# facebookresearch/param

Hardware: AMD Instinct MI355X
Metric: EmbeddingBag lookups/s + achieved HBM GB/s; all-to-all bus-BW at 1/2/4/8 GPU (higher is better)
Workload: dtype f32

## Files before the change

param_amd/csrc/bwd_sorted_apply_impl.inc:

```
__device__ __forceinline__ u32x4 raw16_load(const char* p, int pol) {
    const PM_GLOBAL u32x4* q = as_global<u32x4>(p);
    if (pol == 2) return *reinterpret_cast<const volatile PM_GLOBAL u32x4*>(q);
    return (pol == 1 || pol == 4) ? __builtin_nontemporal_load(q) : *q;
}
__device__ __forceinline__ void raw16_store(char* p, const u32x4 v, int pol) {
    PM_GLOBAL u32x4* q = as_global<u32x4>(p);
#ifdef PM_VISIBLE_STORES
    if (pol == 2) *reinterpret_cast<volatile PM_GLOBAL u32x4*>(q) = v;
    else if (pol >= 3) __hip_atomic_store(reinterpret_cast<PM_GLOBAL uint32_t*>(q), v.x, __ATOMIC_RELAXED, __HIP_MEMORY_SCOPE_AGENT),
                       __hip_atomic_store(reinterpret_cast<PM_GLOBAL uint32_t*>(q) + 1, v.y, __ATOMIC_RELAXED, __HIP_MEMORY_SCOPE_AGENT),
                       __hip_atomic_store(reinterpret_cast<PM_GLOBAL uint32_t*>(q) + 2, v.z, __ATOMIC_RELAXED, __HIP_MEMORY_SCOPE_AGENT),
                       __hip_atomic_store(reinterpret_cast<PM_GLOBAL uint32_t*>(q) + 3, v.w, __ATOMIC_RELAXED, __HIP_MEMORY_SCOPE_AGENT);
    else if (pol == 1) __builtin_nontemporal_store(v, q);
    else *q = v;
    return;
#endif
    if (pol == 2) asm volatile("global_store_dwordx4 %0, %1, off sc0 sc1\n\ts_nop 1" : : "v"(q), "v"(v) : "memory");
    else if (pol >= 3) asm volatile("global_store_dwordx4 %0, %1, off sc1\n\ts_nop 1" : : "v"(q), "v"(v) : "memory");
    else if (pol == 1) asm volatile("global_store_dwordx4 %0, %1, off nt\n\ts_nop 1" : : "v"(q), "v"(v) : "memory");
    else asm volatile("global_store_dwordx4 %0, %1, off\n\ts_nop 1" : : "v"(q), "v"(v) : "memory");
}
__device__ __forceinline__ void hidden_store16(float* p, const float (&a)[4]) {
    const u32x4 v = {__float_as_uint(a[0]), __float_as_uint(a[1]), __float_as_uint(a[2]), __float_as_uint(a[3])};
#ifdef PM_VISIBLE_STORES
// ... 169 lines not shown
        case 16: return launch_apply_w<DST, K, 16>(sp, stream);
        case 32: return launch_apply_w<DST, K, 32>(sp, stream);
        default: return launch_apply_w<DST, K, 64>(sp, stream);
    }
}


template <typename DST>
hipError_t launch_unique_g(const SortedParams& sp, const KParams& kp, const UniqueArgs& ua, int max_dim, hipStream_t stream) {
    unsigned n_wg = static_cast<unsigned>(kp.T) * static_cast<unsigned>(kp.tiles_per_table);
    if (sp.unique_wgs_per_cu > 0 && n_wg > 256u * static_cast<unsigned>(sp.unique_wgs_per_cu)) n_wg = 256u * static_cast<unsigned>(sp.unique_wgs_per_cu);
    const dim3 grid(n_wg), blk(kBlock);
    const size_t lds = tile_lds_bytes(kp.bags_per_block, kp.idx_cap, false);
    const int g = group_lanes(max_dim, DST::kVec);
    if (sp.mom && max_dim > g * DST::kVec) return hipErrorInvalidValue;
#define PM_LAUNCH_UNIQUE(G_)                                                                                                         \
    do {                                                                                                                             \
        if (sp.mom) hipLaunchKernelGGL((bwd_unique_kernel<DST, G_, 1>), grid, blk, lds, stream, sp, kp, ua.hyb_tab, ua.bloom, ua.emit_keys,  \
                                       ua.emit_vals, ua.key_bytes, ua.tile_cnt, ua.tile_cnt_stride, ua.bloom_wbits);                  \
        else hipLaunchKernelGGL((bwd_unique_kernel<DST, G_, 0>), grid, blk, lds, stream, sp, kp, ua.hyb_tab, ua.bloom, ua.emit_keys,         \
                                ua.emit_vals, ua.key_bytes, ua.tile_cnt, ua.tile_cnt_stride, ua.bloom_wbits);                         \
    } while (0)
    switch (g) {
        case 8: PM_LAUNCH_UNIQUE(8); break;
        case 16: PM_LAUNCH_UNIQUE(16); break;
        case 32: PM_LAUNCH_UNIQUE(32); break;
        default: PM_LAUNCH_UNIQUE(64); break;
    }
#undef PM_LAUNCH_UNIQUE
    return hipGetLastError();
}


template <typename DST>
hipError_t launch_rest_g(const SortedParams& sp, const KParams& kp, const RestArgs& ra, int max_dim, hipStream_t stream) {
    if (ra.T_h < 1 || ra.parts < 1) return hipErrorInvalidValue;
    const dim3 grid(static_cast<unsigned>(ra.T_h) * static_cast<unsigned>(ra.parts)), blk(kRestThreads);
    const size_t lds = static_cast<size_t>(2 * kRestCap + kRestAux) * sizeof(uint32_t);
    const int g = group_lanes(max_dim, DST::kVec);
    if (sp.mom && max_dim > g * DST::kVec) return hipErrorInvalidValue;
#define PM_LAUNCH_REST_O(G_, OPT_)                                                                                                  \
    do {                                                                                                                            \
        static const hipError_t attr_ = hipFuncSetAttribute(reinterpret_cast<const void*>(hyb_rest_kernel<DST, G_, OPT_>),          \
                                                            hipFuncAttributeMaxDynamicSharedMemorySize, static_cast<int>(lds));     \
        if (attr_ != hipSuccess) return attr_;                                                                                      \
        hipLaunchKernelGGL((hyb_rest_kernel<DST, G_, OPT_>), grid, blk, lds, stream, sp, kp, ra);                                   \
    } while (0)
#define PM_LAUNCH_REST(G_)                                                    \
    do {                                                                      \
        if (sp.mom) PM_LAUNCH_REST_O(G_, 1); else PM_LAUNCH_REST_O(G_, 0);    \
    } while (0)
    switch (g) {
        case 8: PM_LAUNCH_REST(8); break;
        case 16: PM_LAUNCH_REST(16); break;
        case 32: PM_LAUNCH_REST(32); break;
        default: PM_LAUNCH_REST(64); break;
    }
#undef PM_LAUNCH_REST
#undef PM_LAUNCH_REST_O
    return hipGetLastError();
}
```

param_amd/csrc/embbag_bwd_sorted_kernels.inc:

```

template <typename DST, int G>
__device__ __forceinline__ void adagrad_finish(char* wptr, float (&wrow)[DST::kVec], const float (&acc)[DST::kVec],
                                               bool any_col, float* mom_row, float mom_prev, int D, const SortedParams& p,
                                               int lig, int nt_rows, uint64_t rowkey, int c) {
    float ss = 0.0f;
    if (p.wd_mode == PM_WD_L2) {
#pragma unroll
        for (int k = 0; k < DST::kVec; ++k) {
            const float reg = any_col ? p.wd * wrow[k] : 0.0f;
            const float gx = acc[k] + reg;
            ss = ss + gx * gx;
        }
    } else {
#pragma unroll
        for (int k = 0; k < DST::kVec; ++k) ss = ss + acc[k] * acc[k];
    }
#pragma unroll
    for (int off = G / 2; off >= 1; off >>= 1) ss = ss + __shfl_xor(ss, off, G);
    const float m = mom_prev + ss / static_cast<float>(D);
    if (lig == 0) hidden_store4(mom_row, m);
    const float mult = p.lr / (sqrtf(m) + p.eps);
    if (any_col) {
        if (p.wd_mode != PM_WD_NONE) {
            const float shrink = p.wd_mode == PM_WD_L2 ? mult * p.wd : p.lr * p.wd;
// ... 821 lines not shown
    {
        const PM_GLOBAL uint32_t* sk = as_global<uint32_t>(ra.stage + static_cast<size_t>(t) * 2 * kRestCap);
        const PM_GLOBAL uint32_t* sv = sk + kRestCap;
#pragma unroll
        for (int r = 0; r < kRestItems; ++r) {
            const uint32_t off = static_cast<uint32_t>(r) * kWave + lane, pos = wave * chunk + off;
            const uint32_t e = (off < chunk && pos < n) ? pos : n - 1u;
            key[r] = sk[e];
            val[r] = sv[e];
        }
    }
    PM_STAMP_DRAINED(trace_id, 2);
    const int rounds = (bits + 7) / 8;
    uint32_t* const wcnt = s_aux + wave * 256;
    uint32_t* const s_dstart = s_aux + NW * 256;
    for (int rd = 0; rd < rounds; ++rd) {
        const int shift = 8 * rd;
        const int w = (bits - shift) < 8 ? (bits - shift) : 8;
        const uint32_t mask = (1u << w) - 1u;
        for (int i = threadIdx.x; i < NW * 256; i += kRestThreads) s_aux[i] = 0u;
        __syncthreads();
        uint32_t rank[kRestItems];
#pragma unroll
        for (int r = 0; r < kRestItems; ++r) {
            rank[r] = 0;
            if (static_cast<uint32_t>(r) * kWave < chunk) {
                const uint32_t off = static_cast<uint32_t>(r) * kWave + lane;
                const bool valid = off < chunk && wave * chunk + off < n;
                const uint32_t d = (key[r] >> shift) & mask;
                uint32_t below, total;
                match_digit<8>(d, valid, below, total);
                const uint32_t b0 = valid ? wcnt[d] : 0u;
                rank[r] = b0 + below;
                if (valid && below == 0) wcnt[d] = b0 + total;
            }
        }
        __syncthreads();
        uint32_t acc_d = 0;
        if (threadIdx.x < 256) {
#pragma unroll
            for (int ww = 0; ww < NW; ++ww) {
                const uint32_t c = s_aux[ww * 256 + threadIdx.x];
                s_aux[ww * 256 + threadIdx.x] = acc_d;
                acc_d += c;
            }
        }
        const uint32_t ex = rest_excl_scan<NW>(acc_d, s_tmp);
        if (threadIdx.x < 256) s_dstart[threadIdx.x] = ex;
        __syncthreads();
#pragma unroll
        for (int r = 0; r < kRestItems; ++r) {
            const uint32_t off = static_cast<uint32_t>(r) * kWave + lane;
            if (off < chunk && wave * chunk + off < n) {
                const uint32_t d = (key[r] >> shift) & mask;
                const uint32_t qp = s_dstart[d] + wcnt[d] + rank[r];
                s_key[qp] = key[r];
                s_val[qp] = val[r];
            }
        }
        __syncthreads();
        if (rd + 1 < rounds) {
#pragma unroll
            for (int r = 0; r < kRestItems; ++r) {
                const uint32_t off = static_cast<uint32_t>(r) * kWave + lane, pos = wave * chunk + off;
                if (off < chunk && pos < n) {
                    key[r] = s_key[pos];
                    val[r] = s_val[pos];
// ... 121 lines not shown
```

param_amd/csrc/seg_hybrid.inc:

```

#ifndef PM_MARK_THREADS
#define PM_MARK_THREADS 1024
#endif
constexpr int kMarkThreads = PM_MARK_THREADS;

constexpr int kPartMinSlices = 8;
constexpr int kPartItems = 8;
constexpr int kPartChunk = kMarkThreads * kPartItems;
__device__ __forceinline__ uint32_t part_cap(uint32_t count, int slices) { return count / static_cast<uint32_t>(slices / 2); }

template <int NB>
__global__ void __launch_bounds__(kMarkThreads) hyb_part_kernel(const SegDesc* desc, const HybTable* tab, const void* indices, int idx64, int T_h,
                                                                int64_t n_request, int slices, uint32_t* qa, uint32_t* qb, uint32_t* qtail) {
    constexpr int kW = kMarkThreads / kWave;
    __shared__ uint32_t s_start[kHybMaxTables], s_count[kHybMaxTables];
    __shared__ uint32_t s_sum;
    __shared__ uint32_t s_wcnt[kW][kBloomKMax], s_woff[kW][kBloomKMax], s_base[kBloomKMax];
    if (threadIdx.x == 0) s_sum = 0u;
    __syncthreads();
    {
        const int i = threadIdx.x;
        if (i < T_h) {
            const bool c = tab[i].cand != 0u;
            const SegDesc d = desc[i];
// ... 198 lines not shown
            int32_t v[U];
#pragma unroll
            for (int u = 0; u < U; ++u) {
                const uint32_t i = i0 + u * kMarkThreads + threadIdx.x;
                v[u] = ip[i < n ? i : last];
            }
#pragma unroll
            for (int u = 0; u < U; ++u) visit(static_cast<uint32_t>(v[u]), std::true_type{}, i0 + u * kMarkThreads + threadIdx.x < n);
        }
    }
    PM_STAMP(trace_id, 3);
    wave_lds_fence();
    if (static_cast<uint32_t>(lane) < q_tail - q_head) mark(ring[(q_head + lane) & (kRing - 1)]);
    __syncthreads();
    PM_STAMP(trace_id, 4);
    u32x4* out = reinterpret_cast<u32x4*>(bloom + (static_cast<size_t>(t) * slices + static_cast<size_t>(k)) * kBloomWords);
    const u32x4* d4 = reinterpret_cast<const u32x4*>(dup);
    for (int i = threadIdx.x; i < kBloomWords / 4; i += kMarkThreads) out[i] = d4[i];
    PM_STAMP_DRAINED(trace_id, 5);
}

__device__ __forceinline__ uint32_t bloom_flag(const uint32_t* tmap, uint32_t row, int wbits) {
    const uint32_t mask = bloom_mask(row);
    return (tmap[bloom_word(row, wbits)] & mask) == mask ? 1u : 0u;
}


constexpr int kStagePartsMin = 8, kStagePartsMax = 128;
inline int stage_parts(int tiles_per_table) {
    int p = tiles_per_table / 8;
    return p < kStagePartsMin ? kStagePartsMin : (p > kStagePartsMax ? kStagePartsMax : p);
}

template <typename K>
__global__ void __launch_bounds__(kT) hyb_stage_kernel(SegDesc* desc, HybTable* tab, int T_h, const uint32_t* tile_cnt, size_t cnt_stride,
                                                       HybTiles tl, const K* kb, const uint32_t* vb, K* ka, uint32_t* va, int parts,
                                                       int rest_enable, int tshift, uint32_t* stage, uint32_t* rest_n, uint32_t* stat) {
    __shared__ uint32_t s_tmp[kWaves];
    __shared__ uint32_t s_dst[kCompactMaxTiles + 1];
    const int t = blockIdx.x / parts, part = blockIdx.x % parts;
    if (t >= T_h) return;
    if (tab[t].mode != 1u) {
        if (part == 0 && threadIdx.x == 0) rest_n[t] = 0u;
        return;
    }
    const uint32_t nt = static_cast<uint32_t>(tl.tiles_per_table);
    const uint32_t* tc = tile_cnt + static_cast<size_t>(t) * cnt_stride;
    uint32_t carry = 0;
    for (uint32_t i0 = 0; i0 < nt; i0 += kT) {
        const uint32_t i = i0 + threadIdx.x;
        const uint32_t c = i < nt ? tc[i] : 0u;
        const uint32_t ex = block_excl_scan256(c, s_tmp);
        if (i < nt) s_dst[i] = carry + ex;
        carry += s_tmp[0] + s_tmp[1] + s_tmp[2] + s_tmp[3];
        __syncthreads();
    }
    if (threadIdx.x == 0) s_dst[nt] = carry;
    __syncthreads();
    const uint32_t total = s_dst[nt];
    const bool staged = rest_enable && total <= static_cast<uint32_t>(kRestCap);
    const uint64_t base = desc[t].in_start;
    const uint64_t per_tile = static_cast<uint64_t>(tl.bags_per_tile) * tab[t].pooling;
    const K row_mask = (static_cast<K>(1) << tshift) - 1;
    uint32_t* const st_k = stage + static_cast<size_t>(t) * 2 * kRestCap;
    uint32_t* const st_v = st_k + kRestCap;
    const uint32_t ga = static_cast<uint32_t>(static_cast<uint64_t>(nt) * part / parts), gb = static_cast<uint32_t>(static_cast<uint64_t>(nt) * (part + 1) / parts);
    const uint32_t e0 = s_dst[ga], e1 = s_dst[gb];
    for (uint32_t e = e0 + threadIdx.x; e < e1; e += kT) {
        uint32_t lo = ga, hi = gb;
        while (hi - lo > 1) {
            const uint32_t mid = (lo + hi) >> 1;
            if (s_dst[mid] <= e) lo = mid; else hi = mid;
// ... 24 lines not shown
```

param_amd/csrc/seg_sort.hip:

```cpp
#include <cstdlib>

#include "common.h"
#include "pm_experiments.h"

namespace pm {
namespace {

constexpr int kT = 256;
constexpr int kWaves = kT / kWave;
constexpr int kTile = kSegTile;
constexpr int kTileItems = kTile / kT;
constexpr int kRadix = 256;
constexpr int kRadixMax = 512;
constexpr uint32_t kWaveCap = 1024;
constexpr uint32_t kLocalCap = kTile;
constexpr int kL2Grid = 512;
constexpr int kBuildBags = 1024;
constexpr int kMaxLbPasses = 5;

struct SegHeader {
    uint32_t n_total;
    uint32_t n_tiles;
    uint32_t n_l2;
    uint32_t n_tiles2;
// ... 45 lines not shown
}


__device__ __forceinline__ uint32_t block_excl_scan256(uint32_t v, uint32_t* s_tmp) {
    const int lane = threadIdx.x % kWave, wave = threadIdx.x / kWave;
    uint32_t incl = v;
#pragma unroll
    for (int off = 1; off < kWave; off <<= 1) {
        const uint32_t up = __shfl_up(incl, off, kWave);
        if (lane >= off) incl += up;
    }
    if (lane == kWave - 1) s_tmp[wave] = incl;
    __syncthreads();
    uint32_t base = 0;
    for (int w = 0; w < wave; ++w) base += s_tmp[w];
    __syncthreads();
    return base + incl - v;
}


__global__ void __launch_bounds__(1024) seg_prep_tables_kernel(const void* indices, const void* offsets, int idx64, const int64_t* rows, int T,
                                                               int64_t B, int64_t N, int64_t bag_begin, int64_t bag_count, int force_ragged,
                                                               SegDesc* desc, uint32_t* zero4, const HybArgs hyb, HybTable* hyb_tab, uint32_t* qtail,
                                                               uint32_t* rest_stat) {
    __shared__ uint32_t s_sample[2048];
    __shared__ uint32_t s_rep;
    const int t = blockIdx.x;
    if (zero4 && t == 0 && threadIdx.x < 4) zero4[threadIdx.x] = 0u;
    if (t == 0 && threadIdx.x < 2) rest_stat[threadIdx.x] = 0u;
    if (qtail && t < kHybMaxTables && static_cast<int>(threadIdx.x) < hyb.slices) qtail[static_cast<size_t>(t) * hyb.slices + threadIdx.x] = 0u;
    const int64_t TB = static_cast<int64_t>(T) * B;
    const int64_t g0 = static_cast<int64_t>(t) * B + bag_begin;
    auto off_at = [&](int64_t g) -> int64_t { return g < TB ? load_index(offsets, g, idx64) : N; };
    const int64_t s = off_at(g0);
    const int64_t e = off_at(g0 + bag_count);
    const int64_t cnt = e > s ? e - s : 0;
    const int64_t L = (bag_count > 0 && cnt > 0 && cnt % bag_count == 0) ? cnt / bag_count : 0;
    int bad = (L == 0 || force_ragged) ? 1 : 0;
    const int64_t n_rows = rows[t];
    bool cand = t < kHybMaxTables && !bad && cnt >= kHybMinCount && cnt <= static_cast<int64_t>(hyb.slices) * (kHybMaxCount / kBloomK) &&
                cnt * 4 <= n_rows;
    const bool sample = cand && hyb.allow == 1;
    uint32_t sr[2] = {0u, 0u};
    if (sample) {
        const int64_t stride = cnt / 2048;
#pragma unroll
        for (int u = 0; u < 2; ++u) sr[u] = static_cast<uint32_t>(load_index(indices, s + (threadIdx.x + u * 1024) * stride, idx64));
        for (int i = threadIdx.x; i < 2048; i += 1024) s_sample[i] = 0u;
        if (threadIdx.x == 0) s_rep = 0u;
    }
    if (!bad) {
        for (int64_t i0 = threadIdx.x; i0 < bag_count; i0 += 8 * 1024) {
            int64_t v[8];
#pragma unroll
            for (int u = 0; u < 8; ++u) {
                const int64_t i = i0 + u * 1024;
                v[u] = i < bag_count ? off_at(g0 + i) : s + i * L;
            }
#pragma unroll
            for (int u = 0; u < 8; ++u)
                if (v[u] != s + (i0 + u * 1024) * L) bad = 1;
        }
    }
    bad = __syncthreads_or(bad);
    {
        cand = cand && !bad;
        if (sample) {
            uint32_t rep = 0;
#pragma unroll
            for (int u = 0; u < 2; ++u) {
                const uint32_t h = (sr[u] * 0x9E3779B1u) >> 16;
                rep += (atomicOr(&s_sample[h >> 5], 1u << (h & 31u)) >> (h & 31u)) & 1u;
            }
            if (rep) atomicAdd(&s_rep, rep);
            __syncthreads();
            cand = cand && s_rep * 8u <= 2048u;
        }
        if (threadIdx.x == 0) {
            HybTable h;
            h.mode = 0u;
            h.cand = (cand && hyb.allow) ? 1u : 0u;
            h.pooling = bad ? 0u : static_cast<uint32_t>(L);
            h.n_dup = 0u;
            hyb_tab[t] = h;
        }
    }
    if (threadIdx.x == 0) {
        SegDesc d;
        d.in_start = static_cast<uint32_t>(s);
        d.count = static_cast<uint32_t>(cnt);
        d.out_start = 0;
        d.pooling = bad ? 0u : static_cast<uint32_t>(L);
        d.tile_base = 0;
        d.ntiles = static_cast<uint32_t>((cnt + kTile - 1) / kTile);
        d.rbits = static_cast<uint32_t>(bits_for_dev(static_cast<uint64_t>(rows[t])));
        d.pad = 0;
        desc[t] = d;
    }
}

__device__ __forceinline__ void scan2_1024(uint32_t* s_a, uint32_t* s_b) {
    const int t = threadIdx.x;
    for (int off = 1; off < 1024; off <<= 1) {
        const uint32_t a = t >= off ? s_a[t - off] : 0u;
        const uint32_t b = t >= off ? s_b[t - off] : 0u;
        __syncthreads();
        s_a[t] += a;
        s_b[t] += b;
        __syncthreads();
    }
}

template <typename K, bool WEIGHTED>
__device__ __forceinline__ void build_keys_chunk(int t, int chunk, const void* indices, const void* offsets, int idx64, int T, int64_t B,
                                                 int64_t N, int64_t bag_begin, int64_t bag_count, const SegDesc* desc, int tshift, K* keys,
                                                 uint32_t* vals, uint32_t* bag_of, int64_t* s_off) {
    constexpr int kBags = kBuildBags;
    if (!WEIGHTED && (desc[t].pooling > 0 || desc[t].pad)) return;
    const int64_t bag0 = bag_begin + static_cast<int64_t>(chunk) * kBags;
    const int64_t left = bag_begin + bag_count - bag0;
    if (left <= 0) return;
    const int nb = left < kBags ? static_cast<int>(left) : kBags;
    const int64_t TB = static_cast<int64_t>(T) * B;
    const int64_t g0 = static_cast<int64_t>(t) * B + bag0;
    for (int i = threadIdx.x; i <= nb; i += blockDim.x) s_off[i] = (g0 + i < TB) ? load_index(offsets, g0 + i, idx64) : N;
    __syncthreads();
    const int64_t base = s_off[0], end = s_off[nb];
    for (int64_t j = base + threadIdx.x; j < end; j += blockDim.x) {
        int lo = 0, hi = nb;
        while (hi - lo > 1) {
            const int mid = (lo + hi) >> 1;
            if (s_off[mid] <= j) lo = mid; else hi = mid;
        }
        const uint32_t bag = static_cast<uint32_t>(bag0 + lo);
        keys[j] = (static_cast<K>(t) << tshift) | static_cast<K>(load_index(indices, j, idx64));
        if (WEIGHTED) {
            vals[j] = static_cast<uint32_t>(j);
            bag_of[j] = bag;
        } else {
            vals[j] = bag;
        }
    }
}

template <typename K, bool WEIGHTED>
__global__ void __launch_bounds__(1024) seg_prep_scan_kernel(SegDesc* desc, int T, SegHeader* hdr, TileDesc* tiles, uint32_t tiles_cap,
                                                             const void* indices, const void* offsets, int idx64, int64_t B, int64_t N,
                                                             int64_t bag_begin, int64_t bag_count, int tshift, K* keys, uint32_t* vals,
                                                             uint32_t* bag_of, int chunks_per_table) {
    __shared__ uint32_t s_cnt[1024], s_til[1024], s_tb[1025], s_out[1024];
    __shared__ int64_t s_off[kBuildBags + 1];
    if (blockIdx.x > 0) {
        const int w = static_cast<int>(blockIdx.x) - 1;
        build_keys_chunk<K, WEIGHTED>(w / chunks_per_table, w % chunks_per_table, indices, offsets, idx64, T, B, N, bag_begin, bag_count,
                                      desc, tshift, keys, vals, bag_of, s_off);
        return;
    }
    const int t = threadIdx.x;
    const uint32_t c = t < T ? desc[t].count : 0u;
    const uint32_t nt = t < T ? desc[t].ntiles : 0u;
    s_cnt[t] = c;
    s_til[t] = nt;
    __syncthreads();
    scan2_1024(s_cnt, s_til);
    const uint32_t out_start = s_cnt[t] - c, tile_base = s_til[t] - nt;
    const uint32_t n_total = s_cnt[1023], n_tiles = s_til[1023];
    __syncthreads();
    if (t < T) {
        desc[t].out_start = out_start;
        desc[t].tile_base = tile_base;
        s_tb[t] = tile_base;
        s_out[t] = out_start;
    }
    if (t == 0) {
        s_tb[T] = n_tiles;
        hdr->n_total = n_total;
        hdr->n_tiles = n_tiles;
        hdr->n_l2 = 0;
        hdr->n_tiles2 = 0;
        hdr->lookback_timeouts = 0;
    }
    __syncthreads();
    const uint32_t n_write = n_tiles < tiles_cap ? n_tiles : tiles_cap;
    for (uint32_t g = t; g < n_write; g += 1024) {
        int lo = 0, hi = T;
        while (hi - lo > 1) {
            const int mid = (lo + hi) >> 1;
            if (s_tb[mid] <= g) lo = mid; else hi = mid;
        }
        const SegDesc d = desc[lo];
        const uint32_t first = (g - s_tb[lo]) * static_cast<uint32_t>(kTile);
        TileDesc td;
        td.seg = static_cast<uint32_t>(lo);
        td.cnt = (d.count - first) < static_cast<uint32_t>(kTile) ? d.count - first : static_cast<uint32_t>(kTile);
        td.in_base = d.in_start + first;
        td.out_base = s_out[lo] + first;
        td.first = first;
        td.pooling = d.pooling;
        td.rbits = d.rbits;
        td.magic = d.pooling > 1 ? static_cast<uint32_t>(0x100000000ull / d.pooling) + 1u : 0u;
        tiles[g] = td;
    }
}

template <typename K>
struct PassSrc {
    const void* indices;
    int idx64;
    const K* keys;
    const uint32_t* vals;
    int first;
    int tshift;
    uint32_t bag_begin;
};

__device__ __forceinline__ void wave_hist_add(uint32_t* h, uint32_t dg, bool valid, int lane) {
    const uint64_t vmask = __ballot(valid);
    const uint32_t firstd = __builtin_amdgcn_readfirstlane(dg);
    const bool uniform = __ballot(valid && dg != firstd) == 0 && (vmask & 1ull);
    if (uniform) {
        if (lane == 0) atomicAdd(&h[firstd], static_cast<uint32_t>(__popcll(vmask)));
    } else if (valid) {
        atomicAdd(&h[dg], 1u);
    }
}

template <typename K>
__device__ __forceinline__ void load_tile_rows(const TileDesc& td, const PassSrc<K>& src, uint64_t (&row)[kTileItems]) {
    const uint32_t cnt = td.cnt, last = cnt - 1u;
    auto at = [&](int k) { const uint32_t q = k * kT + threadIdx.x; return q < cnt ? q : last; };
    if (src.first && td.pooling > 0) {
        if (src.idx64) {
            const PM_GLOBAL int64_t* ip = as_global<int64_t>(src.indices) + td.in_base;
#pragma unroll
            for (int k = 0; k < kTileItems; ++k) row[k] = static_cast<uint64_t>(ip[at(k)]);
// ... 343 lines not shown

__device__ __forceinline__ u32x4 load_status(const uint32_t* p) {
    u32x4 v;
    asm volatile("global_load_dwordx4 %0, %1, off sc1\n\ts_waitcnt vmcnt(0)" : "=&v"(v) : "v"(p) : "memory");
    return v;
}
#ifndef PM_LB_BATCH
#define PM_LB_BATCH 4
#endif
constexpr int kLbBatch = PM_LB_BATCH;
__device__ __forceinline__ void load_status_batch(const uint32_t* const (&p)[kLbBatch], u32x4 (&v)[kLbBatch]) {
#if PM_LB_BATCH == 8
    asm volatile(
        "global_load_dwordx4 %0, %8, off sc1\n\tglobal_load_dwordx4 %1, %9, off sc1\n\t"
        "global_load_dwordx4 %2, %10, off sc1\n\tglobal_load_dwordx4 %3, %11, off sc1\n\t"
        "global_load_dwordx4 %4, %12, off sc1\n\tglobal_load_dwordx4 %5, %13, off sc1\n\t"
        "global_load_dwordx4 %6, %14, off sc1\n\tglobal_load_dwordx4 %7, %15, off sc1\n\ts_waitcnt vmcnt(0)"
        : "=&v"(v[0]), "=&v"(v[1]), "=&v"(v[2]), "=&v"(v[3]), "=&v"(v[4]), "=&v"(v[5]), "=&v"(v[6]), "=&v"(v[7])
        : "v"(p[0]), "v"(p[1]), "v"(p[2]), "v"(p[3]), "v"(p[4]), "v"(p[5]), "v"(p[6]), "v"(p[7])
        : "memory");
#else
    asm volatile(
        "global_load_dwordx4 %0, %4, off sc1\n\tglobal_load_dwordx4 %1, %5, off sc1\n\t"
        "global_load_dwordx4 %2, %6, off sc1\n\tglobal_load_dwordx4 %3, %7, off sc1\n\ts_waitcnt vmcnt(0)"
        : "=&v"(v[0]), "=&v"(v[1]), "=&v"(v[2]), "=&v"(v[3])
        : "v"(p[0]), "v"(p[1]), "v"(p[2]), "v"(p[3])
        : "memory");
#endif
}
__device__ __forceinline__ void store_status(uint32_t* p, u32x4 v) {
    asm volatile("global_store_dwordx4 %0, %1, off sc1\n\ts_nop 1" : : "v"(p), "v"(v) : "memory");
}

template <typename K, int RB>
__global__ void __launch_bounds__(kT) seg_hist_all_kernel(const TileDesc* tiles, const uint32_t* n_tiles, const PassSrc<K> src, int npass,
                                                          uint32_t tiles_cap, uint32_t* st) {
    constexpr int RAD = 1 << RB;
    __shared__ uint32_t h[kMaxLbPasses * RAD];
    const TileDesc td = tiles[blockIdx.x];
    const uint32_t nt = *n_tiles;
    if (blockIdx.x >= nt) return;
    const uint32_t g = blockIdx.x, cnt = td.cnt;
    int shift[kMaxLbPasses];
    uint32_t mask[kMaxLbPasses];
#pragma unroll
    for (int p = 0; p < kMaxLbPasses; ++p) pass_digit(0, p, td.rbits, RB, shift[p], mask[p]);
    for (int i = threadIdx.x; i < npass * RAD; i += kT) h[i] = 0;
    __syncthreads();
    const int lane = threadIdx.x % kWave;
    uint64_t row[kTileItems];
    load_tile_rows<K>(td, src, row);
    constexpr uint32_t kNone = 0xffffffffu;
    uint32_t hot0[kMaxLbPasses], hot1[kMaxLbPasses];
#pragma unroll
    for (int p = 0; p < kMaxLbPasses; ++p) {
        hot0[p] = hot1[p] = kNone;
        if (p < npass) {
            const bool v0 = threadIdx.x < cnt;
            const uint32_t dg = static_cast<uint32_t>(row[0] >> shift[p]) & mask[p];
            uint64_t cand = __ballot(v0);
            for (int r = 0; r < 3 && cand != 0; ++r) {
                const int leader = __builtin_amdgcn_readfirstlane(__ffsll(static_cast<long long>(cand)) - 1);
                const uint32_t d0 = __builtin_amdgcn_readlane(dg, leader);
                const uint64_t same = __ballot(v0 && dg == d0);
                cand &= ~same;
                if (__popcll(same) >= 8) {
                    if (hot0[p] == kNone) hot0[p] = d0;
                    else if (hot1[p] == kNone) hot1[p] = d0;
                }
            }
        }
    }
    bool any_hot = false;
#pragma unroll
// ... 515 lines not shown
    return &scratch_layout(const_cast<void*>(scratch), n_max, T).hdr->n_total;
}
const uint32_t* seg_sort_timeouts(const void* scratch, size_t n_max, int T) {
    return &scratch_layout(const_cast<void*>(scratch), n_max, T).hdr->lookback_timeouts;
}
const HybTable* seg_sort_hyb_tab(const void* scratch, size_t n_max, int T) { return scratch_layout(const_cast<void*>(scratch), n_max, T).hyb_tab; }
const uint32_t* seg_sort_bloom(const void* scratch, size_t n_max, int T) { return scratch_layout(const_cast<void*>(scratch), n_max, T).bloom; }
uint32_t* seg_sort_tile_cnt(const void* scratch, size_t n_max, int T) { return scratch_layout(const_cast<void*>(scratch), n_max, T).tile_cnt; }
size_t seg_sort_tile_cnt_stride(size_t n_max) { return tile_cnt_stride(n_max); }
uint32_t* seg_sort_rest_stat(void* scratch, size_t n_max, int T) { return &scratch_layout(scratch, n_max, T).hdr->rest_pairs; }
const uint32_t* seg_sort_rest_stage(const void* scratch, size_t n_max, int T) { return scratch_layout(const_cast<void*>(scratch), n_max, T).rest_stage; }
const uint32_t* seg_sort_rest_n(const void* scratch, size_t n_max, int T) { return scratch_layout(const_cast<void*>(scratch), n_max, T).rest_n; }

int seg_sort_radix_bits(int mode, int rbits_max) {
    if ((mode != 0 && mode != 3) || rbits_max <= 8) return 8;
    return (rbits_max + 8) / 9 < (rbits_max + 7) / 8 ? 9 : 8;
}
int seg_sort_passes(int mode, int rbits_max) {
    if ((mode != 0 && mode != 3) || rbits_max <= 0) return 1;
    const int rb = seg_sort_radix_bits(mode, rbits_max);
    return (rbits_max + rb - 1) / rb;
}
bool seg_sort_result_in_b(int mode, int rbits_max) { return seg_sort_passes(mode, rbits_max) % 2 == 1; }

bool seg_sort_lookback(int mode, int rbits_max, int64_t n) {
    if (mode != 0 || n >= (1ll << 30)) return false;
    const int np = seg_sort_passes(mode, rbits_max);
    return np <= kMaxLbPasses && static_cast<size_t>(np) << seg_sort_radix_bits(mode, rbits_max) <= kLbRowWords;
}

namespace {
template <typename K, int RB>
void launch_lookback(const Scratch& s, unsigned tm, int T, PassSrc<K> src, int total, K* keys_a, K* keys_b, uint32_t* vals_a, uint32_t* vals_b,
                     uint32_t spin_cap, hipStream_t stream) {
    src.first = 1;
    src.keys = keys_a;
    src.vals = vals_a;
    hipLaunchKernelGGL((seg_hist_all_kernel<K, RB>), dim3(tm), dim3(kT), 0, stream, s.tiles, &s.hdr->n_tiles, src, total, tm, s.st_all);
    hipLaunchKernelGGL((seg_scan_all_kernel<RB>), dim3(T, total), dim3(kRadix * kScanChunks), 0, stream, s.desc, s.st_all, tm, T, s.bstart_all);
    for (int p = 0; p < total; ++p) {
        src.first = p == 0 ? 1 : 0;
        src.keys = p == 0 ? keys_a : (p % 2 == 1 ? keys_b : keys_a);
        src.vals = p == 0 ? vals_a : (p % 2 == 1 ? vals_b : vals_a);
        K* kout = (p % 2 == 0) ? keys_b : keys_a;
        uint32_t* vout = (p % 2 == 0) ? vals_b : vals_a;
        hipLaunchKernelGGL((seg_lookback_pass_kernel<K, RB>), dim3(tm), dim3(kT), 0, stream, s.tiles, s.hdr, src, p, T, tm, s.st_all, s.bstart_all,
                           kout, vout, spin_cap);
    }
}
template <typename K, int RB>
void launch_level1_pass(const Scratch& s, unsigned tm, int T, const PassSrc<K>& src, int mode, int p, K* kout, uint32_t* vout, hipStream_t stream) {
    hipLaunchKernelGGL((seg_hist_kernel<K, RB>), dim3(tm), dim3(kT), 0, stream, s.tiles, &s.hdr->n_tiles, src, mode, p, s.bh);
    hipLaunchKernelGGL((seg_scan_kernel<RB>), dim3(T), dim3(kRadix * kScanChunks), 0, stream, s.hdr, s.desc, static_cast<const uint32_t*>(nullptr),
                       static_cast<uint32_t>(T), s.bh, s.bstart, s.bcnt, (mode != 0 && p == 0) ? 1 : 0, mode, s.l2_list);
    hipLaunchKernelGGL((seg_scatter_kernel<K, RB>), dim3(tm), dim3(kT), 0, stream, s.tiles, &s.hdr->n_tiles, src, mode, p, s.bh, s.bstart, kout, vout);
}
}

bool seg_sort_hybrid_available() {
    static const bool ok = hipFuncSetAttribute(reinterpret_cast<const void*>(hyb_mark_kernel), hipFuncAttributeMaxDynamicSharedMemorySize,
                                               2 * kBloomWords * 4) == hipSuccess;
    return ok;
}

template <typename K>
hipError_t seg_sort_part_a(const SegSortRequest& rq, void* scratch, hipStream_t stream) {
    if (rq.N == 0) return hipSuccess;
    if (rq.T < 1 || rq.T > kSegSortMaxTables || rq.N > 0xffffffffLL) return hipErrorInvalidValue;
    const size_t n = static_cast<size_t>(rq.N);
    const Scratch s = scratch_layout(scratch, n, rq.T);
    HybArgs hyb = rq.hyb;
    if (rq.weighted) hyb.allow = 0;
    hipLaunchKernelGGL(seg_prep_tables_kernel, dim3(rq.T), dim3(1024), 0, stream, rq.indices, rq.offsets, rq.idx64, rq.rows, rq.T, rq.B, rq.N,
                       rq.bag_begin, rq.bag_count, rq.weighted ? 1 : 0, s.desc, rq.zero4, hyb, s.hyb_tab, hyb.allow ? s.qtail : nullptr,
                       &s.hdr->rest_pairs);
    if (hyb.allow) {
        if (!seg_sort_hybrid_available()) return hipErrorInvalidValue;
        const int th = rq.T < kHybMaxTables ? rq.T : kHybMaxTables;
        static const int part_env = [] { const char* e = getenv("PARAM_AMD_HYB_PART"); return e ? atoi(e) : -1; }();
        const bool part = rq.queue_a && rq.queue_b && part_env != 0 && (part_env == 1 || hyb.slices >= kPartMinSlices);
        if (part) {
            const unsigned pgrid = static_cast<unsigned>((rq.N + kPartChunk - 1) / kPartChunk);
#define PM_LAUNCH_PART(NB_)                                                                                                               \
    hipLaunchKernelGGL((hyb_part_kernel<NB_>), dim3(pgrid), dim3(kMarkThreads), 0, stream, s.desc, s.hyb_tab, rq.indices, rq.idx64, th, rq.N, \
                       hyb.slices, rq.queue_a, rq.queue_b, s.qtail)
            switch (hyb.slices) {
                case 4: PM_LAUNCH_PART(2); break;
                case 8: PM_LAUNCH_PART(3); break;
                case 16: PM_LAUNCH_PART(4); break;
                case 32: PM_LAUNCH_PART(5); break;
                default: PM_LAUNCH_PART(6); break;
            }
#undef PM_LAUNCH_PART
        }
        const unsigned grid = static_cast<unsigned>(kXcds * hyb.slices * ((th + kXcds - 1) / kXcds));
        hipLaunchKernelGGL(hyb_mark_kernel, dim3(grid), dim3(kMarkThreads), 2 * kBloomWords * 4, stream, s.desc, s.hyb_tab, rq.indices, rq.idx64, th,
                           rq.T, rq.N, s.bloom, hyb.slices, part ? rq.queue_a : nullptr, part ? rq.queue_b : nullptr, part ? s.qtail : nullptr);
    }
    return hipGetLastError();
}

template <typename K>
hipError_t seg_sort_stage_leftovers(const SegSortRequest& rq, const K* keys_b, const uint32_t* vals_b, K* keys_a, uint32_t* vals_a,
                                    HybTiles tiles, int rest_enable, void* scratch, hipStream_t stream) {
    if (rq.N == 0) return hipSuccess;
    if (rq.T < 1 || rq.T > kSegSortMaxTables || rq.N > 0xffffffffLL) return hipErrorInvalidValue;
    if (tiles.tiles_per_table < 1 || tiles.tiles_per_table > kCompactMaxTiles) return hipErrorInvalidValue;
    const size_t n = static_cast<size_t>(rq.N);
    const Scratch s = scratch_layout(scratch, n, rq.T);
    const int th = rq.T < kHybMaxTables ? rq.T : kHybMaxTables;
    const int parts = stage_parts(tiles.tiles_per_table);
    hipLaunchKernelGGL((hyb_stage_kernel<K>), dim3(th * parts), dim3(kT), 0, stream, s.desc, s.hyb_tab, th, s.tile_cnt, tile_cnt_stride(n), tiles,
                       keys_b, vals_b, keys_a, vals_a, parts, rest_enable, rq.tshift, s.rest_stage, s.rest_n, &s.hdr->rest_pairs);
    return hipGetLastError();
}

template <typename K>
hipError_t seg_sort_part_b(const SegSortRequest& rq, int mode, K* keys_a, K* keys_b, uint32_t* vals_a, uint32_t* vals_b, uint32_t* bag_of,
                           void* scratch, hipStream_t stream, bool hybrid_done) {
    if (rq.N == 0) return hipSuccess;
    if (rq.T < 1 || rq.T > kSegSortMaxTables || rq.N > 0xffffffffLL) return hipErrorInvalidValue;
    const size_t n = static_cast<size_t>(rq.N);
    const Scratch s = scratch_layout(scratch, n, rq.T);
    const unsigned tm = static_cast<unsigned>(tiles_max(n, rq.T));
    if (rq.hyb.allow && !rq.weighted && !hybrid_done) return hipErrorInvalidValue;
    {
        const int chunks = rq.bag_count > 0 ? static_cast<int>((rq.bag_count + kBuildBags - 1) / kBuildBags) : 0;
        const dim3 gp(1u + static_cast<unsigned>(chunks) * static_cast<unsigned>(rq.T));
        if (rq.weighted)
            hipLaunchKernelGGL((seg_prep_scan_kernel<K, true>), gp, dim3(1024), 0, stream, s.desc, rq.T, s.hdr, s.tiles, tm, rq.indices,
                               rq.offsets, rq.idx64, rq.B, rq.N, rq.bag_begin, rq.bag_count, rq.tshift, keys_a, vals_a, bag_of, chunks);
        else
            hipLaunchKernelGGL((seg_prep_scan_kernel<K, false>), gp, dim3(1024), 0, stream, s.desc, rq.T, s.hdr, s.tiles, tm, rq.indices,
                               rq.offsets, rq.idx64, rq.B, rq.N, rq.bag_begin, rq.bag_count, rq.tshift, keys_a, vals_a, bag_of, chunks);
    }
    const int total = seg_sort_passes(mode, rq.rbits_max), rb = seg_sort_radix_bits(mode, rq.rbits_max);
    const bool lookback = seg_sort_lookback(mode, rq.rbits_max, rq.N);
    if (mode == 3) mode = 0;
    PassSrc<K> src;
    src.indices = rq.indices;
    src.idx64 = rq.idx64;
    src.tshift = rq.tshift;
    src.bag_begin = static_cast<uint32_t>(rq.bag_begin);
    if (lookback) {
        const uint32_t cap = rq.spin_cap ? rq.spin_cap : kLbSpinCap;
        if (rb == 9) launch_lookback<K, 9>(s, tm, rq.T, src, total, keys_a, keys_b, vals_a, vals_b, cap, stream);
        else launch_lookback<K, 8>(s, tm, rq.T, src, total, keys_a, keys_b, vals_a, vals_b, cap, stream);
        return hipGetLastError();
    }
    for (int p = 0; p < total; ++p) {
        src.first = p == 0 ? 1 : 0;
        src.keys = p == 0 ? keys_a : (p % 2 == 1 ? keys_b : keys_a);
        src.vals = p == 0 ? vals_a : (p % 2 == 1 ? vals_b : vals_a);
        K* kout = (p % 2 == 0) ? keys_b : keys_a;
        uint32_t* vout = (p % 2 == 0) ? vals_b : vals_a;
        if (rb == 9) launch_level1_pass<K, 9>(s, tm, rq.T, src, mode, p, kout, vout, stream);
        else launch_level1_pass<K, 8>(s, tm, rq.T, src, mode, p, kout, vout, stream);
    }
    if (mode != 0 && rq.rbits_max > 8) {
        const uint32_t nb = static_cast<uint32_t>(rq.T) * kRadix;
        hipLaunchKernelGGL((seg_local_kernel<K>), dim3((nb + kWaves - 1) / kWaves), dim3(kT), 0, stream, s.desc, s.bstart, s.bcnt, nb, mode,
                           keys_b, vals_b);
        hipLaunchKernelGGL(seg_l2_prep_kernel, dim3(1), dim3(1024), 0, stream, s.hdr, s.desc, s.bstart, s.bcnt, s.l2_list, mode, s.desc2,
                           static_cast<uint32_t>(seg2_max(n)), s.tiles2, static_cast<uint32_t>(tiles2_max(n)));
        int p2 = (rq.rbits_max - 8 + 7) / 8;
        if (p2 % 2) ++p2;
        src.first = 0;
        for (int q = 0; q < p2; ++q) {
            src.keys = (q % 2 == 0) ? keys_b : keys_a;
            src.vals = (q % 2 == 0) ? vals_b : vals_a;
            K* kout = (q % 2 == 0) ? keys_a : keys_b;
            uint32_t* vout = (q % 2 == 0) ? vals_a : vals_b;
            hipLaunchKernelGGL((seg_hist_kernel<K, 8>), dim3(kL2Grid), dim3(kT), 0, stream, s.tiles2, &s.hdr->n_tiles2, src, 0, q, s.bh2);
            hipLaunchKernelGGL((seg_scan_kernel<8>), dim3(kL2Grid / 2), dim3(kRadix * kScanChunks), 0, stream, s.hdr, s.desc2, &s.hdr->n_l2, 0u, s.bh2, s.bstart2,
                               s.bcnt2, 0, 0, static_cast<uint32_t*>(nullptr));
            hipLaunchKernelGGL((seg_scatter_loop_kernel<K, 8>), dim3(kL2Grid), dim3(kT), 0, stream, s.tiles2, &s.hdr->n_tiles2, src, 0, q, s.bh2,
                               s.bstart2, kout, vout);
        }
    }
    return hipGetLastError();
// ... 25 lines not shown
```

Before: 21.86 billion.

## Fuse key-build into hybrid stage kernel and self-compute tile descriptors in histogram

Unweighted key-building work moves into extra blocks of the hybrid stage kernel. When lookback sort is used, the histogram kernel derives the tile descriptors itself through an in-block scan, so the separate prep/scan launch is dropped. This is meant to remove kernel launches and serialization in the sorted backward path. It also makes the shared-memory attribute cache per device, prefetches the first offsets in the pooling check, and adds LDS fences around the radix rank update. The cost is redundant per-block descriptor scans and more complex control flow; an environment variable can turn the fusion off.

```diff
diff --git a/param_amd/csrc/bwd_sorted_apply_impl.inc b/param_amd/csrc/bwd_sorted_apply_impl.inc
--- a/param_amd/csrc/bwd_sorted_apply_impl.inc
+++ b/param_amd/csrc/bwd_sorted_apply_impl.inc
@@ -225,6 +225,7 @@
 }
 
 
+constexpr int kRestAttrDevices = 64;
 template <typename DST>
 hipError_t launch_rest_g(const SortedParams& sp, const KParams& kp, const RestArgs& ra, int max_dim, hipStream_t stream) {
     if (ra.T_h < 1 || ra.parts < 1) return hipErrorInvalidValue;
@@ -232,11 +233,17 @@
     const size_t lds = static_cast<size_t>(2 * kRestCap + kRestAux) * sizeof(uint32_t);
     const int g = group_lanes(max_dim, DST::kVec);
     if (sp.mom && max_dim > g * DST::kVec) return hipErrorInvalidValue;
+    int dev = 0;
+    if (hipGetDevice(&dev) != hipSuccess || dev < 0) return hipErrorInvalidDevice;
 #define PM_LAUNCH_REST_O(G_, OPT_)                                                                                                  \
     do {                                                                                                                            \
-        static const hipError_t attr_ = hipFuncSetAttribute(reinterpret_cast<const void*>(hyb_rest_kernel<DST, G_, OPT_>),          \
-                                                            hipFuncAttributeMaxDynamicSharedMemorySize, static_cast<int>(lds));     \
-        if (attr_ != hipSuccess) return attr_;                                                                                      \
+        static unsigned char set_[kRestAttrDevices];                                                                                \
+        if (dev >= kRestAttrDevices || !__atomic_load_n(&set_[dev], __ATOMIC_ACQUIRE)) {                                            \
+            const hipError_t attr_ = hipFuncSetAttribute(reinterpret_cast<const void*>(hyb_rest_kernel<DST, G_, OPT_>),             \
+                                                         hipFuncAttributeMaxDynamicSharedMemorySize, static_cast<int>(lds));        \
+            if (attr_ != hipSuccess) return attr_;                                                                                  \
+            if (dev < kRestAttrDevices) __atomic_store_n(&set_[dev], static_cast<unsigned char>(1), __ATOMIC_RELEASE);              \
+        }                                                                                                                           \
         hipLaunchKernelGGL((hyb_rest_kernel<DST, G_, OPT_>), grid, blk, lds, stream, sp, kp, ra);                                   \
     } while (0)
 #define PM_LAUNCH_REST(G_)                                                    \
diff --git a/param_amd/csrc/embbag_bwd_sorted_kernels.inc b/param_amd/csrc/embbag_bwd_sorted_kernels.inc
--- a/param_amd/csrc/embbag_bwd_sorted_kernels.inc
+++ b/param_amd/csrc/embbag_bwd_sorted_kernels.inc
@@ -877,7 +877,9 @@
                 match_digit<8>(d, valid, below, total);
                 const uint32_t b0 = valid ? wcnt[d] : 0u;
                 rank[r] = b0 + below;
+                wave_lds_fence();
                 if (valid && below == 0) wcnt[d] = b0 + total;
+                wave_lds_fence();
             }
         }
         __syncthreads();
diff --git a/param_amd/csrc/seg_hybrid.inc b/param_amd/csrc/seg_hybrid.inc
--- a/param_amd/csrc/seg_hybrid.inc
+++ b/param_amd/csrc/seg_hybrid.inc
@@ -254,12 +254,29 @@
     return p < kStagePartsMin ? kStagePartsMin : (p > kStagePartsMax ? kStagePartsMax : p);
 }
 
+constexpr int kStageBuildBags = 256;
+struct StageBuild {
+    const void* indices;
+    const void* offsets;
+    int idx64, T, chunks;
+    int64_t B, N, bag_begin, bag_count;
+};
 template <typename K>
 __global__ void __launch_bounds__(kT) hyb_stage_kernel(SegDesc* desc, HybTable* tab, int T_h, const uint32_t* tile_cnt, size_t cnt_stride,
                                                        HybTiles tl, const K* kb, const uint32_t* vb, K* ka, uint32_t* va, int parts,
-                                                       int rest_enable, int tshift, uint32_t* stage, uint32_t* rest_n, uint32_t* stat) {
+                                                       int rest_enable, int tshift, uint32_t* stage, uint32_t* rest_n, uint32_t* stat,
+                                                       const StageBuild bld) {
     __shared__ uint32_t s_tmp[kWaves];
-    __shared__ uint32_t s_dst[kCompactMaxTiles + 1];
+    __shared__ __attribute__((aligned(16))) uint32_t s_dst[kCompactMaxTiles + 1];
+    if (static_cast<int>(blockIdx.x) >= T_h * parts) {
+        int64_t* const s_off = reinterpret_cast<int64_t*>(s_dst);
+        static_assert(sizeof(s_dst) >= (kStageBuildBags + 1) * sizeof(int64_t), "the offsets fit the scan's array");
+        const int w = static_cast<int>(blockIdx.x) - T_h * parts, tb = w / bld.chunks;
+        if (tb >= bld.T) return;
+        build_keys_chunk<K, false, kStageBuildBags>(tb, w % bld.chunks, bld.indices, bld.offsets, bld.idx64, bld.T, bld.B, bld.N, bld.bag_begin,
+                                                    bld.bag_count, tab[tb].pooling > 0u, tshift, ka, va, nullptr, s_off);
+        return;
+    }
     const int t = blockIdx.x / parts, part = blockIdx.x % parts;
     if (t >= T_h) return;
     if (tab[t].mode != 1u) {
diff --git a/param_amd/csrc/seg_sort.hip b/param_amd/csrc/seg_sort.hip
--- a/param_amd/csrc/seg_sort.hip
+++ b/param_amd/csrc/seg_sort.hip
@@ -101,6 +101,12 @@
     const int64_t TB = static_cast<int64_t>(T) * B;
     const int64_t g0 = static_cast<int64_t>(t) * B + bag_begin;
     auto off_at = [&](int64_t g) -> int64_t { return g < TB ? load_index(offsets, g, idx64) : N; };
+    int64_t v0[8];
+#pragma unroll
+    for (int u = 0; u < 8; ++u) {
+        const int64_t i = static_cast<int64_t>(threadIdx.x) + u * 1024;
+        v0[u] = i < bag_count ? off_at(g0 + i) : 0;
+    }
     const int64_t s = off_at(g0);
     const int64_t e = off_at(g0 + bag_count);
     const int64_t cnt = e > s ? e - s : 0;
@@ -119,7 +125,12 @@
         if (threadIdx.x == 0) s_rep = 0u;
     }
     if (!bad) {
-        for (int64_t i0 = threadIdx.x; i0 < bag_count; i0 += 8 * 1024) {
+#pragma unroll
+        for (int u = 0; u < 8; ++u) {
+            const int64_t i = static_cast<int64_t>(threadIdx.x) + u * 1024;
+            if (i < bag_count && v0[u] != s + i * L) bad = 1;
+        }
+        for (int64_t i0 = static_cast<int64_t>(threadIdx.x) + 8 * 1024; i0 < bag_count; i0 += 8 * 1024) {
             int64_t v[8];
 #pragma unroll
             for (int u = 0; u < 8; ++u) {
@@ -180,12 +191,12 @@
     }
 }
 
-template <typename K, bool WEIGHTED>
+template <typename K, bool WEIGHTED, int BAGS = kBuildBags>
 __device__ __forceinline__ void build_keys_chunk(int t, int chunk, const void* indices, const void* offsets, int idx64, int T, int64_t B,
-                                                 int64_t N, int64_t bag_begin, int64_t bag_count, const SegDesc* desc, int tshift, K* keys,
+                                                 int64_t N, int64_t bag_begin, int64_t bag_count, bool skip, int tshift, K* keys,
                                                  uint32_t* vals, uint32_t* bag_of, int64_t* s_off) {
-    constexpr int kBags = kBuildBags;
-    if (!WEIGHTED && (desc[t].pooling > 0 || desc[t].pad)) return;
+    constexpr int kBags = BAGS;
+    if (!WEIGHTED && skip) return;
     const int64_t bag0 = bag_begin + static_cast<int64_t>(chunk) * kBags;
     const int64_t left = bag_begin + bag_count - bag0;
     if (left <= 0) return;
@@ -221,8 +232,10 @@
     __shared__ int64_t s_off[kBuildBags + 1];
     if (blockIdx.x > 0) {
         const int w = static_cast<int>(blockIdx.x) - 1;
-        build_keys_chunk<K, WEIGHTED>(w / chunks_per_table, w % chunks_per_table, indices, offsets, idx64, T, B, N, bag_begin, bag_count,
-                                      desc, tshift, keys, vals, bag_of, s_off);
+        const int tb = w / chunks_per_table;
+        const bool skip = !WEIGHTED && (desc[tb].pooling > 0 || desc[tb].pad);
+        build_keys_chunk<K, WEIGHTED>(tb, w % chunks_per_table, indices, offsets, idx64, T, B, N, bag_begin, bag_count, skip, tshift, keys,
+                                      vals, bag_of, s_off);
         return;
     }
     const int t = threadIdx.x;
@@ -270,6 +283,95 @@
         td.magic = d.pooling > 1 ? static_cast<uint32_t>(0x100000000ull / d.pooling) + 1u : 0u;
         tiles[g] = td;
     }
+}
+
+constexpr int kSelfPer = kSegSortMaxTables / kT;
+constexpr int kSelfWords = 2 * kWaves + 10;
+static_assert(kSelfPer * kT == kSegSortMaxTables, "every table of the largest request has a thread");
+__device__ __forceinline__ bool self_tile_desc(SegDesc* desc, int T, SegHeader* hdr, TileDesc* tiles, uint32_t* s_tb, uint32_t* s_x,
+                                               TileDesc& td) {
+    const int lane = threadIdx.x % kWave, wave = threadIdx.x / kWave;
+    const int i0 = static_cast<int>(threadIdx.x) * kSelfPer;
+    SegDesc d[kSelfPer];
+#pragma unroll
+    for (int k = 0; k < kSelfPer; ++k) {
+        d[k] = desc[i0 + k < T ? i0 + k : T - 1];
+        if (i0 + k >= T) d[k].count = d[k].ntiles = 0u;
+    }
+    uint32_t sc = 0, sn = 0;
+#pragma unroll
+    for (int k = 0; k < kSelfPer; ++k) { sc += d[k].count; sn += d[k].ntiles; }
+    uint32_t ic = sc, in = sn;
+#pragma unroll
+    for (int o = 1; o < kWave; o <<= 1) {
+        const uint32_t uc = __shfl_up(ic, o, kWave), un = __shfl_up(in, o, kWave);
+        if (lane >= o) { ic += uc; in += un; }
+    }
+    if (lane == kWave - 1) { s_x[wave] = ic; s_x[kWaves + wave] = in; }
+    __syncthreads();
+    uint32_t ec = ic - sc, en = in - sn, n_total = 0, n_tiles = 0;
+#pragma unroll
+    for (int w = 0; w < kWaves; ++w) {
+        if (w < wave) { ec += s_x[w]; en += s_x[kWaves + w]; }
+        n_total += s_x[w];
+        n_tiles += s_x[kWaves + w];
+    }
+    uint32_t out0[kSelfPer], tb0[kSelfPer];
+#pragma unroll
+    for (int k = 0; k < kSelfPer; ++k) {
+        out0[k] = ec;
+        tb0[k] = en;
+        s_tb[i0 + k] = en;
+        ec += d[k].count;
+        en += d[k].ntiles;
+    }
+    if (blockIdx.x == 0) {
+#pragma unroll
+        for (int k = 0; k < kSelfPer; ++k)
+            if (i0 + k < T) {
+                desc[i0 + k].out_start = out0[k];
+                desc[i0 + k].tile_base = tb0[k];
+            }
+        if (threadIdx.x == 0) {
+            hdr->n_total = n_total;
+            hdr->n_tiles = n_tiles;
+            hdr->n_l2 = 0;
+            hdr->n_tiles2 = 0;
+            hdr->lookback_timeouts = 0;
+        }
+    }
+    const uint32_t g = blockIdx.x;
+    if (g >= n_tiles) return false;
+    __syncthreads();
+    int lo = 0, hi = T;
+    while (hi - lo > 1) {
+        const int mid = (lo + hi) >> 1;
+        if (s_tb[mid] <= g) lo = mid; else hi = mid;
+    }
+    uint32_t* const s_td = s_x + 2 * kWaves;
+    if (lo / kSelfPer == static_cast<int>(threadIdx.x)) {
+#pragma unroll
+        for (int k = 0; k < kSelfPer; ++k)
+            if (lo % kSelfPer == k) {
+                const uint32_t first = (g - tb0[k]) * static_cast<uint32_t>(kTile);
+                TileDesc x;
+                x.seg = static_cast<uint32_t>(lo);
+                x.cnt = (d[k].count - first) < static_cast<uint32_t>(kTile) ? d[k].count - first : static_cast<uint32_t>(kTile);
+                x.in_base = d[k].in_start + first;
+                x.out_base = out0[k] + first;
+                x.first = first;
+                x.pooling = d[k].pooling;
+                x.rbits = d[k].rbits;
+                x.magic = d[k].pooling > 1 ? static_cast<uint32_t>(0x100000000ull / d[k].pooling) + 1u : 0u;
+                tiles[g] = x;
+                s_td[0] = x.seg; s_td[1] = x.cnt; s_td[2] = x.in_base; s_td[3] = x.out_base;
+                s_td[4] = x.first; s_td[5] = x.pooling; s_td[6] = x.rbits; s_td[7] = x.magic;
+            }
+    }
+    __syncthreads();
+    td.seg = s_td[0]; td.cnt = s_td[1]; td.in_base = s_td[2]; td.out_base = s_td[3];
+    td.first = s_td[4]; td.pooling = s_td[5]; td.rbits = s_td[6]; td.magic = s_td[7];
+    return true;
 }
 
 template <typename K>
@@ -679,14 +781,21 @@
     asm volatile("global_store_dwordx4 %0, %1, off sc1\n\ts_nop 1" : : "v"(p), "v"(v) : "memory");
 }
 
-template <typename K, int RB>
-__global__ void __launch_bounds__(kT) seg_hist_all_kernel(const TileDesc* tiles, const uint32_t* n_tiles, const PassSrc<K> src, int npass,
-                                                          uint32_t tiles_cap, uint32_t* st) {
+template <typename K, int RB, bool SELF>
+__global__ void __launch_bounds__(kT) seg_hist_all_kernel(TileDesc* tiles, const uint32_t* n_tiles, const PassSrc<K> src, int npass,
+                                                          uint32_t tiles_cap, uint32_t* st, SegDesc* desc, int T, SegHeader* hdr) {
     constexpr int RAD = 1 << RB;
+    static_assert(kMaxLbPasses * RAD >= kSegSortMaxTables, "the histogram's words hold the scanned tile bases first");
     __shared__ uint32_t h[kMaxLbPasses * RAD];
-    const TileDesc td = tiles[blockIdx.x];
-    const uint32_t nt = *n_tiles;
-    if (blockIdx.x >= nt) return;
+    TileDesc td;
+    if constexpr (SELF) {
+        __shared__ uint32_t s_self[kSelfWords];
+        if (!self_tile_desc(desc, T, hdr, tiles, h, s_self, td)) return;
+    } else {
+        td = tiles[blockIdx.x];
+        const uint32_t nt = *n_tiles;
+        if (blockIdx.x >= nt) return;
+    }
     const uint32_t g = blockIdx.x, cnt = td.cnt;
     int shift[kMaxLbPasses];
     uint32_t mask[kMaxLbPasses];
@@ -1268,11 +1377,16 @@
 namespace {
 template <typename K, int RB>
 void launch_lookback(const Scratch& s, unsigned tm, int T, PassSrc<K> src, int total, K* keys_a, K* keys_b, uint32_t* vals_a, uint32_t* vals_b,
-                     uint32_t spin_cap, hipStream_t stream) {
+                     uint32_t spin_cap, bool self_desc, hipStream_t stream) {
     src.first = 1;
     src.keys = keys_a;
     src.vals = vals_a;
-    hipLaunchKernelGGL((seg_hist_all_kernel<K, RB>), dim3(tm), dim3(kT), 0, stream, s.tiles, &s.hdr->n_tiles, src, total, tm, s.st_all);
+    if (self_desc)
+        hipLaunchKernelGGL((seg_hist_all_kernel<K, RB, true>), dim3(tm), dim3(kT), 0, stream, s.tiles, &s.hdr->n_tiles, src, total, tm, s.st_all,
+                           s.desc, T, s.hdr);
+    else
+        hipLaunchKernelGGL((seg_hist_all_kernel<K, RB, false>), dim3(tm), dim3(kT), 0, stream, s.tiles, &s.hdr->n_tiles, src, total, tm, s.st_all,
+                           s.desc, T, s.hdr);
     hipLaunchKernelGGL((seg_scan_all_kernel<RB>), dim3(T, total), dim3(kRadix * kScanChunks), 0, stream, s.desc, s.st_all, tm, T, s.bstart_all);
     for (int p = 0; p < total; ++p) {
         src.first = p == 0 ? 1 : 0;
@@ -1291,6 +1405,11 @@
                        static_cast<uint32_t>(T), s.bh, s.bstart, s.bcnt, (mode != 0 && p == 0) ? 1 : 0, mode, s.l2_list);
     hipLaunchKernelGGL((seg_scatter_kernel<K, RB>), dim3(tm), dim3(kT), 0, stream, s.tiles, &s.hdr->n_tiles, src, mode, p, s.bh, s.bstart, kout, vout);
 }
+}
+
+static bool prep_fused() {
+    static const bool on = [] { const char* e = getenv("PARAM_AMD_PREP_FUSE"); return !(e && e[0] == '0'); }();
+    return on;
 }
 
 bool seg_sort_hybrid_available() {
@@ -1346,8 +1465,19 @@
     const Scratch s = scratch_layout(scratch, n, rq.T);
     const int th = rq.T < kHybMaxTables ? rq.T : kHybMaxTables;
     const int parts = stage_parts(tiles.tiles_per_table);
-    hipLaunchKernelGGL((hyb_stage_kernel<K>), dim3(th * parts), dim3(kT), 0, stream, s.desc, s.hyb_tab, th, s.tile_cnt, tile_cnt_stride(n), tiles,
-                       keys_b, vals_b, keys_a, vals_a, parts, rest_enable, rq.tshift, s.rest_stage, s.rest_n, &s.hdr->rest_pairs);
+    StageBuild bld;
+    bld.indices = rq.indices;
+    bld.offsets = rq.offsets;
+    bld.idx64 = rq.idx64;
+    bld.T = rq.T;
+    bld.chunks = (prep_fused() && rq.bag_count > 0) ? static_cast<int>((rq.bag_count + kStageBuildBags - 1) / kStageBuildBags) : 0;
+    bld.B = rq.B;
+    bld.N = rq.N;
+    bld.bag_begin = rq.bag_begin;
+    bld.bag_count = rq.bag_count;
+    const unsigned grid = static_cast<unsigned>(th * parts) + static_cast<unsigned>(bld.chunks) * static_cast<unsigned>(rq.T);
+    hipLaunchKernelGGL((hyb_stage_kernel<K>), dim3(grid), dim3(kT), 0, stream, s.desc, s.hyb_tab, th, s.tile_cnt, tile_cnt_stride(n), tiles,
+                       keys_b, vals_b, keys_a, vals_a, parts, rest_enable, rq.tshift, s.rest_stage, s.rest_n, &s.hdr->rest_pairs, bld);
     return hipGetLastError();
 }
 
@@ -1360,8 +1490,11 @@
     const Scratch s = scratch_layout(scratch, n, rq.T);
     const unsigned tm = static_cast<unsigned>(tiles_max(n, rq.T));
     if (rq.hyb.allow && !rq.weighted && !hybrid_done) return hipErrorInvalidValue;
-    {
-        const int chunks = rq.bag_count > 0 ? static_cast<int>((rq.bag_count + kBuildBags - 1) / kBuildBags) : 0;
+    const bool lookback = seg_sort_lookback(mode, rq.rbits_max, rq.N);
+    const bool built = hybrid_done && rq.hyb.allow && !rq.weighted && prep_fused();
+    const bool self_desc = built && lookback;
+    if (!self_desc) {
+        const int chunks = built ? 0 : rq.bag_count > 0 ? static_cast<int>((rq.bag_count + kBuildBags - 1) / kBuildBags) : 0;
         const dim3 gp(1u + static_cast<unsigned>(chunks) * static_cast<unsigned>(rq.T));
         if (rq.weighted)
             hipLaunchKernelGGL((seg_prep_scan_kernel<K, true>), gp, dim3(1024), 0, stream, s.desc, rq.T, s.hdr, s.tiles, tm, rq.indices,
@@ -1371,7 +1504,6 @@
                                rq.offsets, rq.idx64, rq.B, rq.N, rq.bag_begin, rq.bag_count, rq.tshift, keys_a, vals_a, bag_of, chunks);
     }
     const int total = seg_sort_passes(mode, rq.rbits_max), rb = seg_sort_radix_bits(mode, rq.rbits_max);
-    const bool lookback = seg_sort_lookback(mode, rq.rbits_max, rq.N);
     if (mode == 3) mode = 0;
     PassSrc<K> src;
     src.indices = rq.indices;
@@ -1380,8 +1512,8 @@
     src.bag_begin = static_cast<uint32_t>(rq.bag_begin);
     if (lookback) {
         const uint32_t cap = rq.spin_cap ? rq.spin_cap : kLbSpinCap;
-        if (rb == 9) launch_lookback<K, 9>(s, tm, rq.T, src, total, keys_a, keys_b, vals_a, vals_b, cap, stream);
-        else launch_lookback<K, 8>(s, tm, rq.T, src, total, keys_a, keys_b, vals_a, vals_b, cap, stream);
+        if (rb == 9) launch_lookback<K, 9>(s, tm, rq.T, src, total, keys_a, keys_b, vals_a, vals_b, cap, self_desc, stream);
+        else launch_lookback<K, 8>(s, tm, rq.T, src, total, keys_a, keys_b, vals_a, vals_b, cap, self_desc, stream);
         return hipGetLastError();
     }
     for (int p = 0; p < total; ++p) {
```

After: 22.04 billion, median of 2. No clear change (+0.8%).
